# RoboEden/flatland-marl

Measured on AMD Instinct MI355X. Metric: agent-steps/sec (batched envs) + tree-obs build ms/step, higher is better.
Workload: dtype int32; 1 GPU; cfg2: 256 envs x 30x30 / 20 agents / 3 cities (Round-2 Test_2); envs_per_gpu=256, agents=20, obs=cutils(31 nodes, pred 500) + upstream tree depth 2 (pred 30), actions=counter-hash uniform 0..4 generated on device, auto-reset at episode end, distinct_maps=8, dm_rebuild=at commit only, parallelism=envs sharded over 1 GPU(s), metrics all-reduce only, launch=one host call per kernel launch

## Files before the change

flatland_marl_amd/csrc/fl_obs_body.h:

```cpp
#pragma once
#include "fl_obs_trees.h"

__device__ __forceinline__ int obs_env_of_workgroup(const FlObsScratch &S) { return __builtin_amdgcn_readfirstlane(S.order ? S.order[blockIdx.x] : (int)blockIdx.x); }

template <bool CUTILS, int VAR, int STAGE, int MERGED = 0, int FIX = 0, bool UP = true>
__device__ __forceinline__ void obs_body(const FlDev &d, const FlObsScratch &S, const ObsArgs &P_launch) {
    using FixT = ObsFixed<FIX != 0 ? FIX : 1>;
    ObsArgs P_local = P_launch;
    if (FIX != 0) {
        P_local.max_nodes = FixT::max_nodes; P_local.pred_depth = FixT::pred_depth; P_local.tree_pred = FixT::shape.tree_pred;
        P_local.tshift = obs_fixed_tshift<FIX != 0 ? FIX : 1>(d.A);
        if (FixT::max_depth != 0) {
            P_local.max_depth = FixT::max_depth;
            P_local.n_tree_nodes = FixT::max_depth == 2 ? 21 : 85;
        }
    }
    const ObsArgs &P = P_local;
    constexpr bool TAB_LDS = (VAR & 1) != 0, WL_HBM = (VAR & 2) != 0;
    const int b = MERGED == 1 ? (int)blockIdx.x : obs_env_of_workgroup(S), tid = threadIdx.x,
              nt = MERGED == 3 ? 512 : (FIX != 0 || MERGED == 1 || MERGED == 2) ? OBS_NT : (int)blockDim.x;
    const int A = (FIX != 0 && FixT::agents != 0) ? FixT::agents : d.A, R = d.R[b], NS = R * 4, K = d.K[b], U = d.U[b];
    const int Rcap = d.Rcap, Scap = Rcap * 4;
    const int lane = tid & 63, wave = tid >> 6;

// ... 352 lines not shown
            } else va |= 1u << ACT_NOTHING;
        } else if (state == ST_READY) va = (1u << ACT_FORWARD) | (1u << ACT_STOP);
        else va = 1u << ACT_NOTHING;
        if (gl < 5) out_store(&P.valid[(size_t)g * 5 + gl], (uint8_t)((va >> gl) & 1));
        if (P.props && gl == 5) {
            out_store(&P.props[(size_t)g * 3 + 0], (double)dist_target);
            out_store(&P.props[(size_t)g * 3 + 2], (double)(state == ST_READY));
        }
        const int road_type = raw.road_type;
        const uint32_t malfw = raw.malfw;
        const uint32_t malf01 = (malfw & 0xFFFFu) != 0, nmalf01 = (malfw >> 16) != 0;
        const uint32_t rev = __brev(cell) >> 16;
        unsigned long long m_lo = (state < 7u ? 1ull << state : 0ull) | (road_type < 11 ? 1ull << (7 + road_type) : 0ull) | (1ull << (18 + nmalf01)) |
                                  (1ull << (28 + init_dir)) | (1ull << (32 + dir)) | (1ull << (36 + old_dir)) |
                                  ((unsigned long long)(state == ST_MOVING) << 40) | ((unsigned long long)PK_SIGMALF(pk) << 42) |
                                  ((unsigned long long)(!malf01) << 43) | ((unsigned long long)(scount == 0) << 44) |
                                  ((unsigned long long)(scount == max_count) << 45) | ((unsigned long long)(state == ST_MALF || state == ST_MALF_OFF) << 46) |
                                  ((unsigned long long)is_off_map(state) << 47) | ((unsigned long long)is_on_map(state) << 48) |
                                  ((unsigned long long)(rev & 0x7FFFu) << 49);
        const uint32_t m_hi = (rev >> 15) | (va << 1);
        const float max_t = (float)T, max_dist_target = (float)((d.H + d.W) * 8);
        const float f_step = (float)tnow / max_t;
        const float f_latest = (float)raw.latest / max_t;
        const float f_before = f_latest - f_step;
        const float f_dist = isinf(dist_target) ? 8.0f : dist_target / max_dist_target;
        const float fv[13] = {(float)i / (float)A, f_step, (float)raw.earliest / max_t, f_latest, (float)raw.arrival / max_t, f_before, f_dist,
                              f_before < f_dist ? f_before : f_dist, (float)max_count / 10, (float)a_speed[i] / 1.0f, (float)scount / 10,
                              (float)malf01 / 10, isinf(init_dist) ? 8.0f : init_dist / max_dist_target};
        float *o = P.attr + (size_t)g * FL_CUTILS_ATTR;
        out_store(&o[gl], (float)((m_lo >> gl) & 1ull));
        if (gl + 32 != 41) out_store(&o[gl + 32], (float)((m_lo >> (gl + 32)) & 1ull));
        if (gl + 64 < FL_CUTILS_ATTR) {
            float v = (float)((m_hi >> gl) & 1u);
#pragma unroll
            for (int k = 0; k < 13; k++) v = gl == 6 + k ? fv[k] : v;
            out_store(&o[gl + 64], v);
        }
    };
    auto phase1b_all = [&]() __attribute__((always_inline)) {
        for (int i = wave * 2 + (lane >> 5); i < A; i += 2 * (nt >> 6)) phase1b(i, lane & 31, phase1b_load(i));
    };

    const bool do_p1 = CUTILS && STAGE != 2;
    const int nw_walk = (X.Tn > 0 && STAGE != 2) ? min((nt >> 6) - ((do_p1 && (nt >> 6) > 4) ? 1 : 0), max(2, (A + 7) / 8)) : 0;
    const bool p1_beside_walk = nw_walk < (nt >> 6);
    const int n_p1_all = (do_p1 && p1_beside_walk && X.Tn > 0) ? (A + 1) / 2 : 0;
    const bool late_p1 = merged && n_p1_all > 0;
    const int n_up_jobs = (merged && UP) ? (min(A, ROUND) + 3) / 4 : 0, n_p1_jobs = late_p1 ? 0 : n_p1_all;
    constexpr int PF_CHUNK = 64 * 16;
    const int pf_n2 = bg_prefill ? A * P.n_tree_nodes * 6 : 0, n_pf_jobs = (pf_n2 + PF_CHUNK - 1) / PF_CHUNK;
    auto drain_jobs = [&]() __attribute__((always_inline)) {
        bool stored = false;
        while (n_up_jobs + n_p1_jobs + n_pf_jobs > 0) {
            int j = 0;
            if (lane == 0) j = atomicAdd(&misc[6], 1);
            j = __builtin_amdgcn_readfirstlane(j);
            if (j >= n_up_jobs + n_p1_jobs + n_pf_jobs) break;
            if (j < n_up_jobs) {
                const int u = 4 * j + (lane >> 4);
                upstream_pass_a<16, OBS_CAP_T_COMPACT, true, 32>(X, P, b, u, u < A, lane & 15, merged_table_t<ROUND>(wave_scr, min(u, ROUND - 1)), &d.err[b]);
            } else if (j < n_up_jobs + n_p1_jobs) {
                const int i = 2 * (j - n_up_jobs) + (lane >> 5);
                if (i < A) phase1b(i, lane & 31, phase1b_load(i));
            } else {
                double2 *o2 = reinterpret_cast<double2 *>(P.tree_out + (size_t)b * A * P.n_tree_nodes * 12);
                const double2 ninf = make_double2(-INFINITY, -INFINITY);
                const int k0 = (j - n_up_jobs - n_p1_jobs) * PF_CHUNK + lane;
#pragma unroll
                for (int q = 0; q < 16; q++)
                    if (k0 + q * 64 < pf_n2) fill_store_d2(reinterpret_cast<double *>(o2 + k0 + q * 64), -INFINITY, -INFINITY);
                stored = true;
            }
        }
        if (stored) asm volatile("s_waitcnt vmcnt(0)" ::: "memory");
    };
    constexpr bool TOPO_JOBS = MERGED == 1 && OBS_TOPO_JOBS;
    auto late_jobs = [&](bool after_barrier = false) __attribute__((always_inline)) {
        while (late_p1 && !(TOPO_JOBS && after_barrier)) {
            int j = 0;
            if (lane == 0) j = atomicAdd(&misc[7], 1);
            j = __builtin_amdgcn_readfirstlane(j);
            if (j >= n_p1_all) break;
            const int i = 2 * j + (lane >> 5);
            if (i < A) phase1b(i, lane & 31, phase1b_load(i));
        }
        while (TOPO_JOBS && (after_barrier || P.no_early_topo == 0)) {
            int j = 0;
            if (lane == 0) j = atomicAdd(&misc[5], 1);
            j = __builtin_amdgcn_readfirstlane(j);
            if (2 * j >= min(A, 32)) break;
            const int t = 2 * j + (lane >> 5);
            const bool have_t = t < A;
            cutils_rows_orders<OBS_CAP_C, !UP, 1>(X, d, P, b, t, have_t, lane & 31, merged_table_c(wave_scr, min(t, 31)),
                                                  have_t ? team_meta[64 + t] : 1, have_t ? team_meta[192 + t] : 0, (float)T);
        }
    };
    if (do_p1 && (!p1_beside_walk || X.Tn == 0)) {
        if (wave == 0) phase1a();
        phase1b_all();
        __syncthreads();
    }
    OBS_STAMP(2);
    if (X.Tn > 0) {
        const bool dual = UP && CUTILS && STAGE == 1 && p_dual_index && P.tree_pred >= 0;
        const bool reuse = STAGE == 2 && p_dual_index && misc[4] != 0;
        const int Tn2 = P.tree_pred + 1, tshift2 = Tn2 <= 64 ? 0 : P.tshift;
        const bool bk = CUTILS && STAGE != 2 && p_bk != 0 && X.Tn > 64 && X.tmask != nullptr;
        const bool bk_lds = bk && p_bk == 2;
        const int bk_nb = p_bk_nb, bk_shift = p_bk_shift;
        const int bk_w = bk_lds ? bk_nb + 2 : bk_nb;
        uint32_t *bkc = bk_lds ? LDS_AT(uint32_t, L_BKREL) : reinterpret_cast<uint32_t *>(wave_scr);
        if (!reuse) {
            for (int k = tid; k <= K; k += nt) csr[k] = 0;
            if (tid == 0) misc[11] = 0;
            if (X.tmask) for (int k = tid; k <= K; k += nt) { tmask[k] = 0ull; if (X.tmask_m2) tmask_m2[k] = 0ull; }
            if (cmask) for (int k = tid; k < NS; k += nt) cmask[k] = 0ull;
            if (bk) for (int k = tid; k < (bk_lds ? K * bk_w / 2 : ((K + 1) * bk_nb + 1) / 2); k += nt) bkc[k] = 0u;
        }
        if (dual) for (int k = tid; k <= K; k += nt) { csr2[k] = 0; if (p_use_tmask) tmaskb[k] = 0ull; if (X.tmask_m2) tmaskb_m2[k] = 0ull; }
        if (dual && cmaskb) for (int k = tid; k < NS; k += nt) cmaskb[k] = 0u;
        if (STAGE != 2 && tid < 64) { team_meta[64 + tid] = 1; team_meta[192 + tid] = 1; }
        __syncthreads();
        const int pred_depth = my_pred_depth;
        if (STAGE != 2) {
        const int w_first = (nt >> 6) - nw_walk, wsel = wave - w_first;
        if (do_p1 && p1_beside_walk && wave == w_first - 1) {
            phase1a();
#ifdef FL_OBS_TIMING
            if (lane == 0) atomicMax((unsigned long long *)&X.dbg[20], (unsigned long long)wall_clock64());
#endif
        }
        if (wsel >= 0) __builtin_amdgcn_s_setprio(3);
        const int n_max = CUTILS ? pred_depth + 1 : max(pred_depth, 1);
        for (int base = 0; wsel >= 0 && base < A; base += 8 * nw_walk) {
            const int slot = lane >> 3, j = lane & 7;
            const int i = base + wsel * 8 + slot;
            const bool have = i < A;
            const int ia = have ? i : 0;
            uint16_t *path = S.path + ((size_t)b * A + ia) * OBS_PRED_CAP;
            const int u = a_tslot[ia];
            uint32_t st = ((uint32_t)a_vpos[ia] << 2) | a_dir[ia];
            bool alive = have && j < n_max;
            auto lead_in = [&](const uint16_t *nh_u) __attribute__((always_inline)) {
                for (int h = 0; h < 7; h++) {
                    if (alive && h < j) {
                        const uint32_t hop = ((uint32_t)nh_u[st >> 2] >> (3u * (st & 3u))) & 7u;
                        const uint32_t nr = hop == 4u ? (uint32_t)FL_R_NONE : (uint32_t)nbr[(st & ~3u) | hop];
                        if (nr == FL_R_NONE) alive = false;
                        else st = (nr << 2) | hop;
                    }
                }
            };
            const bool listed = !lab || lab[ia] >= 0;
            const int hz1 = ((bk && !bk_lds) || !listed) ? -1 : max(0, CUTILS ? (X.Tn - 2) / (int)a_tpc[ia] + 1 : (X.Tn - 1) / (int)a_tpc[ia]);
            const int tpc_w = a_tpc[ia], tlast_w = X.Tn - 1;
            uint32_t st_hz = 0;
            const int hz2 = dual ? max(0, min(P.tree_pred - 1, (Tn2 - 1) / (int)a_tpc2[ia])) : -1;
            auto walk8 = [&](const uint16_t *h8) __attribute__((always_inline)) {
                int idx = j, last = -1;
                while (__any(alive)) {
                    if (alive) {
                        path[idx] = (uint16_t)st;
                        last = idx;
                        if (idx <= hz1 || idx <= hz2) {
                            const int key = key_of(X, (int)(st >> 2));
                            if (idx <= hz1) {
                                if (bk_lds) {
                                    const int tlo = idx == 0 ? 0 : (idx - 1) * tpc_w + 1, thi = min(idx * tpc_w, tlast_w);
                                    const int b1 = min(tlo >> bk_shift, bk_nb - 1), b2 = min(thi >> bk_shift, bk_nb - 1);
                                    for (int bb = b1; bb <= b2; bb++) {
                                        const int kb = key * bk_w + bb;
                                        atomicAdd(&bkc[kb >> 1], (kb & 1) ? 0x10000u : 1u);
                                    }
                                    atomicAdd(&csr[key], b2 - b1 + 1);
                                    if (idx == hz1) st_hz = st;
                                } else {
                                    atomicAdd(&csr[key], 1);
                                }
                            }
                            if (idx <= hz2) atomicAdd(&csr2[key], 1);
                        }
                        const uint32_t s8 = idx + 8 < n_max ? (uint32_t)h8[st] : (uint32_t)FL_R_NONE;
                        if (s8 == FL_R_NONE) alive = false;
                        else { st = s8; idx += 8; }
                    }
                }
                return last;
            };
            if (nh_in_lds) lead_in(nh_lds + u * Rcap);
            else lead_in(gnh + (size_t)u * Rcap);
            const int my_last = TAB_LDS ? walk8(hop8_lds + u * Scap) : walk8(ghop8 + (size_t)u * Scap);
            int m = my_last;
            m = max(m, __shfl_xor(m, 1)); m = max(m, __shfl_xor(m, 2)); m = max(m, __shfl_xor(m, 4));
            if (bk_lds && have && listed) {
                const int lp = max(0, min(m, hz1));
                if (lp == m ? my_last == lp : j == (lp & 7)) {
                    const uint32_t s_lp = lp == m ? st : st_hz;
                    const int key = key_of(X, (int)(s_lp >> 2));
                    const int tlo = lp == 0 ? 0 : (lp - 1) * tpc_w + 1, thi = min(lp * tpc_w, tlast_w);
                    const int b1 = min(tlo >> bk_shift, bk_nb - 1), b2 = min(thi >> bk_shift, bk_nb - 1);
                    for (int bb = b1; bb <= b2; bb++) {
                        const int kb = key * bk_w + bb;
                        atomicSub(&bkc[kb >> 1], (kb & 1) ? 0x10000u : 1u);
                    }
                    atomicAdd(&bkc[(key * bk_w + bk_nb) >> 1], 1u);
                    atomicOr(&bkc[(key * bk_w + bk_nb) >> 1], 0x10000u << (b1 >> OBS_FB_MSHIFT));
                    if (b2 > b1) atomicSub(&csr[key], b2 - b1);
                }
            }
            if (have && j == 0) {
                const int n = m + 1;
                const int tpc = a_tpc[i];
                const int horizon = CUTILS ? (X.Tn - 2) / tpc + 1 : (X.Tn - 1) / tpc;
                a_lp[i] = (uint16_t)max(0, min(n - 1, horizon));
                a_n[i] = (uint16_t)n;
                if (dual) {
                    const int tpc2 = a_tpc2[i];
                    const int n_py = (n - 1 < P.tree_pred) ? n : P.tree_pred;
                    a_lp2[i] = (uint16_t)max(0, min(n_py - 1, (Tn2 - 1) / tpc2));
                }
            }
        }
        if (wsel >= 0) __builtin_amdgcn_s_setprio(0);
#ifdef FL_OBS_TIMING
        if (wsel >= 0 && lane == 0) atomicMax((unsigned long long *)&X.dbg[21], (unsigned long long)wall_clock64());
#endif
        {
#ifdef FL_OBS_TIMING
            const long long t_pa0 = (long long)wall_clock64();
#endif
            if (CUTILS && (!bk || bk_lds) && P.max_nodes <= OBS_CAP_C) {
                const int n_first = min(A, merged ? ROUND : (nt >> 6) * 2);
                auto hoisted = [&](auto team_tag) __attribute__((always_inline)) {
                    constexpr int TEAM = decltype(team_tag)::value;
                    const int grp = lane / TEAM, gl = lane % TEAM, team_id = wave * (64 / TEAM) + grp;
                    if (__builtin_amdgcn_readfirstlane(wave * (64 / TEAM)) >= n_first) return;
                    int node_base, levels;
                    const bool have = team_id < n_first;
                    cutils_pass_a<OBS_CAP_C, TEAM>(X, d, P, b, team_id, have, grp, gl,
                                  merged ? merged_table_c(wave_scr, min(team_id, ROUND - 1)) : wave_scr + min(team_id, min((nt >> 6) * 2, A)) * (N_WORDS_C * OBS_CAP_C),
                                  a_vpos, a_pos, a_dir, a_state, a_speed, a_tslot, (float)T,
                                  a_raw ? a_raw[(have ? team_id : 0) * 8 + 1] : d.spk[b * A + (have ? team_id : 0)],
                                  a_raw ? a_raw[(have ? team_id : 0) * 8 + 2] : d.malf[b * A + (have ? team_id : 0)], node_base, levels);
                    if (gl == 0 && have) { team_meta[64 + team_id] = node_base; team_meta[192 + team_id] = levels; }
                };
                if (p_compact_t) hoisted(std::integral_constant<int, 16>());
                else hoisted(std::integral_constant<int, 32>());
            }
#ifdef FL_OBS_TIMING
            if (lane == 0) {
                atomicMax((unsigned long long *)&X.dbg[19], (unsigned long long)wall_clock64());
                atomicMax((unsigned long long *)&X.dbg[23], (unsigned long long)((long long)wall_clock64() - t_pa0));
            }
#endif
            drain_jobs();
        }
#ifdef FL_OBS_TIMING
        if (lane == 0) atomicMax((unsigned long long *)&X.dbg[22], (unsigned long long)wall_clock64());
#endif
        if (bk && !bk_lds) {
            __syncthreads();
            for (int i = wave; i < A; i += (nt >> 6)) {
                if (lab && lab[i] < 0) continue;
                const uint16_t *path = S.path + ((size_t)b * A + i) * OBS_PRED_CAP;
                const int lp = a_lp[i];
                const int tpc = a_tpc[i], tlast = X.Tn - 1;
                for (int k0 = lane; k0 <= lp; k0 += 256) {
                    uint32_t wv[4];
#pragma unroll
                    for (int q = 0; q < 4; q++) wv[q] = path[min(k0 + 64 * q, lp)];
#pragma unroll
                    for (int q = 0; q < 4; q++) {
                        const int k = k0 + 64 * q;
                        if (k > lp) break;
                        const int key = key_of(X, (int)(wv[q] >> 2));
                        const int tlo = k == 0 ? 0 : (k - 1) * tpc + 1, span = k == 0 ? 1 : tpc;
                        const int thi = (k == lp || tlo + span - 1 >= tlast) ? tlast : tlo + span - 1;
                        const int b1 = min(tlo >> bk_shift, bk_nb - 1), b2 = min(thi >> bk_shift, bk_nb - 1);
                        for (int bb = b1; bb <= b2; bb++) {
                            const int kb = bb * (K + 1) + key + 1;
                            atomicAdd(&bkc[kb >> 1], (kb & 1) ? 0x10000u : 1u);
                        }
                    }
                }
            }
        }
        } else if (!reuse) {
            for (int i = tid; i < A; i += nt) {
                const int n_c = a_n[i];
                const int n_py = (n_c - 1 < pred_depth) ? n_c : pred_depth;
                const int horizon = (X.Tn - 1) / a_tpc[i];
                a_lp[i] = (uint16_t)max(0, min(n_py - 1, horizon));
            }
            __syncthreads();
            for (int i = wave; i < A; i += (nt >> 6)) {
                const uint16_t *path = S.path + ((size_t)b * A + i) * OBS_PRED_CAP;
                const int lp = a_lp[i];
                for (int k = lane; k <= lp; k += 64) atomicAdd(&csr[key_of(X, (int)(path[k] >> 2))], 1);
            }
        }
        __syncthreads();
        OBS_STAMP(3);
        const bool bk_major = bk && !bk_lds;
        if (!reuse && !bk_major) {
            const int chunk = (K + 1 + nt - 1) / nt;
            const int lo = min(tid * chunk, K + 1), hi = min(lo + chunk, K + 1);
            int sum = 0;
            int longest = 0;
            for (int k = lo; k < hi; k++) {
                sum += dual ? (csr[k] | (csr2[k] << 16)) : csr[k];
                longest = max(longest, dual ? max(csr[k], csr2[k]) : csr[k]);
            }
            if (longest > CF_DIRECT && !bk) misc[11] = 1;
            partial[tid] = sum;
            __syncthreads();
            if (wave == 0) {
                constexpr int PER = OBS_NT / 64;
                const int per = nt >> 6;
                int loc[PER], tot = 0;
#pragma unroll
                for (int q = 0; q < PER; q++) { loc[q] = q < per ? partial[lane * per + q] : 0; tot += loc[q]; }
                const int incl = wave_incl_scan<64>(tot);
                int run = incl - tot;
#pragma unroll
                for (int q = 0; q < PER; q++) { if (q < per) partial[lane * per + q] = run; run += loc[q]; }
            }
            __syncthreads();
            int run = partial[tid];
            if (dual) {
                for (int k = lo; k < hi; k++) {
                    const int v = csr[k] | (csr2[k] << 16);
                    csr[k] = run & 0xFFFF; csr2[k] = (int)((unsigned)run >> 16);
                    run += v;
                }
                if (hi == K + 1 && lo < hi) { misc[2] = run & 0xFFFF; misc[3] = (int)((unsigned)run >> 16); }
            } else {
                for (int k = lo; k < hi; k++) { const int v = csr[k]; csr[k] = run; run += v; }
                if (hi == K + 1 && lo < hi) misc[2] = run;
            }
        }
        if (bk_major) {
            uint16_t *c16 = reinterpret_cast<uint16_t *>(bkc);
            const int K1 = K + 1, n = K1 * bk_nb;
            {
                int most = 0;
                for (int key = tid; key < K; key += nt) {
                    int prev = 0;
                    for (int bb = 0; bb < bk_nb; bb++) { const int c = c16[bb * K1 + key + 1]; most = max(most, prev + c); prev = c; }
                }
                if (most > CF_DIRECT) misc[11] = 1;
            }
            const int chunk = (n + nt - 1) / nt;
            const int lo = min(tid * chunk, n), hi = min(lo + chunk, n);
            int sum = 0;
            for (int k = lo; k < hi; k++) sum += c16[k];
            partial[tid] = sum;
            __syncthreads();
            if (wave == 0) {
                constexpr int PER = OBS_NT / 64;
                const int per = nt >> 6;
                int loc[PER], tot = 0;
#pragma unroll
                for (int q = 0; q < PER; q++) { loc[q] = q < per ? partial[lane * per + q] : 0; tot += loc[q]; }
                const int incl = wave_incl_scan<64>(tot);
                int run = incl - tot;
#pragma unroll
                for (int q = 0; q < PER; q++) { if (q < per) partial[lane * per + q] = run; run += loc[q]; }
            }
            __syncthreads();
            {
                int run = partial[tid];
                for (int k = lo; k < hi; k++) {
                    if (k % K1 == 0) misc[12 + k / K1] = run;
                    run += c16[k];
                }
                if (hi == n && lo < hi) misc[2] = run;
            }
            __syncthreads();
            {
                int run = partial[tid], row = lo / K1, rbase = lo < n ? misc[12 + row] : 0, next = (row + 1) * K1;
                for (int k = lo; k < hi; k++) {
                    if (k == next) { row++; rbase = misc[12 + row]; next += K1; }
                    const int c = c16[k];
                    c16[k] = (uint16_t)(run - rbase);
                    run += c;
                }
            }
        }
        __syncthreads();
        if (reuse) {
            csr = csr2; X.csr_end = csr2; X.items_lds = items2;
            X.tmask = p_use_tmask ? tmaskb : nullptr;
            if (!X.tmask) { X.wl_occ_cap = wl_entries; X.wl_cf = X.wl_occ + X.wl_occ_cap; X.wl_cf_cap = 0; }
        }
        if (bk_lds) {
            for (int key = tid; key < K; key += nt) {
                uint32_t *w4 = bkc + key * (bk_w / 2);
                uint32_t run = 0, prev = 0, most = 0;
                for (int q = 0; q < bk_nb / 2; q++) {
                    const uint32_t v = w4[q], c0 = v & 0xFFFFu, c1 = v >> 16;
                    most = max(most, max(prev + c0 + c1, c0 + c1));
                    prev = c0 + c1;
                    w4[q] = run | ((run + c0) << 16);
                    run += c0 + c1;
                }
                if (bk_lds) {
                    const uint32_t ve = w4[bk_nb / 2];
                    w4[bk_nb / 2] = run | (ve & 0xFFFF0000u);
                    most += ve & 0xFFFFu;
                }
                if (most > CF_DIRECT) misc[11] = 1;
            }
            __syncthreads();
        }
#ifdef FL_OBS_TIMING
        if (STAGE != 2) { __syncthreads(); if (tid == 0) P.dbg[(size_t)b * 64 + 56] = (long long)wall_clock64(); }
#endif
        const bool fit = items_lds != nullptr && misc[2] <= L_FIELD(items_cap);
        const bool dual_fill = dual && misc[3] <= L_FIELD(items2_cap);
        if (dual && tid == 0) misc[4] = dual_fill ? 1 : 0;
        if (merged && UP && !dual_fill) atomicCAS(&d.err[b], 0, FL_ERR_CAPACITY);
        if (fit && !reuse) { csr_items = items_lds; X.items_lds = items_lds; }
        constexpr int FU = 4;
#ifdef OBS_NO_LEAN_FILL
        constexpr bool LEAN_FILL = false;
#else
        constexpr bool LEAN_FILL = MERGED == 1;
#endif
        uint32_t pfv[FU] = {0, 0, 0, 0}, pfn[FU] = {0, 0, 0, 0}, pfp[FU] = {0, 0, 0, 0};
        auto prefetch = [&](int ia) __attribute__((always_inline)) {
            if (reuse || ia >= A) return;
            const uint16_t *pth = S.path + ((size_t)b * A + ia) * OBS_PRED_CAP;
            const int lpn = a_lp[ia];
#pragma unroll
            for (int q = 0; q < FU; q++) {
                const int k = min(lane + 64 * q, lpn);
                pfv[q] = pth[k]; pfn[q] = pth[min(k + 1, lpn)]; pfp[q] = pth[max(k - 1, 0)];
            }
        };
        if (bk_major) {
            const int K1 = K + 1, tlast = X.Tn - 1;
            uint16_t *pre16 = reinterpret_cast<uint16_t *>(partial);
            uint16_t *klo16 = pre16 + ((A + 2) & ~1);
            for (int bb = 0; bb < bk_nb; bb++) {
                const int t0 = bb << bk_shift, t1 = bb == bk_nb - 1 ? tlast : min(t0 + (1 << bk_shift) - 1, tlast);
                if (t0 > tlast) break;
                const int gbase = misc[12 + bb];
                for (int ia = tid; ia < A; ia += nt) {
                    const int lp = a_lp[ia], tpc = a_tpc[ia];
                    const int k_lo = min((t0 + tpc - 1) / tpc, lp);
                    const int k_hi = min(t1 >= 1 ? (t1 - 1) / tpc + 1 : 0, lp);
                    klo16[ia] = (uint16_t)k_lo;
                    pre16[ia + 1] = (lab && lab[ia] < 0) ? (uint16_t)0 : (uint16_t)(k_hi - k_lo + 1);
                }
                if (tid == 0) pre16[0] = 0;
                __syncthreads();
                if (wave == 0) {
                    const int per = (A + 63) >> 6, a_lo = min(lane * per, A), a_hi = min(a_lo + per, A);
                    int sum = 0;
                    for (int ia = a_lo; ia < a_hi; ia++) sum += pre16[ia + 1];
                    int run = wave_incl_scan<64>(sum) - sum;
                    for (int ia = a_lo; ia < a_hi; ia++) { run += pre16[ia + 1]; pre16[ia + 1] = (uint16_t)run; }
                }
                __syncthreads();
                const int total = pre16[A];
                uint32_t nv = 0, nn = 0, np = 0;
                int n_i = 0, n_k = 0;
                auto request = [&](int t) __attribute__((always_inline)) {
                    if (t >= total) return;
                    int lo_a = 0, hi_a = A - 1;
                    while (lo_a < hi_a) {
                        const int mid = (lo_a + hi_a + 1) >> 1;
                        if ((int)pre16[mid] <= t) lo_a = mid; else hi_a = mid - 1;
                    }
                    n_i = lo_a;
                    n_k = (int)klo16[lo_a] + (t - (int)pre16[lo_a]);
                    const uint16_t *pth = S.path + ((size_t)b * A + lo_a) * OBS_PRED_CAP;
                    const int lp = a_lp[lo_a];
                    nv = pth[n_k]; nn = pth[min(n_k + 1, lp)]; np = pth[max(n_k - 1, 0)];
                };
                request(tid);
                for (int t = tid; t < total; t += nt) {
                    const int i = n_i, k = n_k;
                    const uint32_t w = nv, wnx = nn, wpv = np;
                    request(t + nt);
                    const int lp = a_lp[i], tpc = a_tpc[i];
                    const int tlo = k == 0 ? 0 : (k - 1) * tpc + 1, span = k == 0 ? 1 : tpc;
                    const bool to_end = k == lp || tlo + span - 1 >= tlast;
                    const int thi = to_end ? tlast : tlo + span - 1;
                    const int b1 = min(tlo >> bk_shift, bk_nb - 1), b2 = min(thi >> bk_shift, bk_nb - 1);
                    if (bb < b1 || bb > b2) continue;
                    const int key = key_of(X, (int)(w >> 2));
                    if (X.tmask && bb == b1) {
                        const int m1 = tb_of(tlo, X.tshift), m2 = tb_of(thi, X.tshift);
                        atomicOr(&tmask[key], ((2ull << m2) - 1ull) & ~((1ull << m1) - 1ull));
                    }
                    const uint32_t dnext = k < lp ? (wnx & 3u) : (w & 3u), dprev = k > 0 ? (wpv & 3u) : (w & 3u);
                    const uint32_t item = IT_MAKE(lab ? (int)lab[i] : i, tlo, to_end, span, dprev, dnext, w & 3u);
                    const int kb = bb * K1 + key + 1;
                    const uint32_t old = atomicAdd(&bkc[kb >> 1], (kb & 1) ? 0x10000u : 1u);
                    csr_items[gbase + (int)((kb & 1) ? (old >> 16) : (old & 0xFFFFu))] = item;
                }
                __syncthreads();
            }
        }
        prefetch(bk_major ? A : wave);
        for (int i = wave; !reuse && !bk_major && i < A; i += (nt >> 6)) {
            const uint16_t *path = S.path + ((size_t)b * A + i) * OBS_PRED_CAP;
            const int lp = (lab && lab[i] < 0) ? -1 : (int)a_lp[i], tpc = a_tpc[i], tlast = X.Tn - 1;
            const int lp2 = dual_fill ? (int)a_lp2[i] : -1, tpc2 = dual_fill ? (int)a_tpc2[i] : 1;
            uint32_t wv[FU], wnx[FU], wpv[FU];
#pragma unroll
            for (int q = 0; q < FU; q++) { wv[q] = pfv[q]; wnx[q] = pfn[q]; wpv[q] = pfp[q]; }
            prefetch(i + (nt >> 6));
            for (int k0 = lane; k0 <= lp; k0 += 64 * FU) {
            if (k0 != lane) {
#pragma unroll
                for (int q = 0; q < FU; q++) {
                    const int k = min(k0 + 64 * q, lp);
                    wv[q] = path[k]; wnx[q] = path[min(k + 1, lp)]; wpv[q] = path[max(k - 1, 0)];
                }
            }
#pragma unroll
            for (int q = 0; q < FU; q++) {
                const int k = k0 + 64 * q;
                if (k > lp) break;
                const uint32_t w = wv[q];
                const uint32_t dnext = k < lp ? (wnx[q] & 3u) : (w & 3u), dprev = k > 0 ? (wpv[q] & 3u) : (w & 3u);
                int tlo, span;
                if (CUTILS) {
                    tlo = k == 0 ? 0 : (k - 1) * tpc + 1;
                    span = k == 0 ? 1 : tpc;
                } else {
                    tlo = k * tpc;
                    span = tpc;
                }
                const bool to_end = k == lp || tlo + span - 1 >= tlast;
                const int key = key_of(X, (int)(w >> 2));
                if (LEAN_FILL) {
                    const int b1 = tb_of(tlo, X.tshift), b2 = tb_of(to_end ? tlast : tlo + span - 1, X.tshift);
                    const unsigned long long bits = ((2ull << b2) - 1ull) & ~((1ull << b1) - 1ull);
                    const bool second = k <= lp2, done = a_state[i] == ST_DONE;
                    const int tlo2 = k * tpc2, tlast2 = Tn2 - 1;
                    const bool to_end2 = k == lp2 || tlo2 + tpc2 - 1 >= tlast2;
                    unsigned long long bits2 = 0ull, seen = 0ull, seen2 = 0ull;
                    int slot2 = 0;
                    if (X.tmask && X.tmask_m2) seen = atomicOr(&tmask[key], bits);
                    else if (X.tmask) atomicOr(&tmask[key], bits);
                    if (second) {
                        if (p_use_tmask) {
                            const int c1 = tb_of(tlo2, tshift2), c2 = tb_of(to_end2 ? tlast2 : tlo2 + tpc2 - 1, tshift2);
                            bits2 = ((2ull << c2) - 1ull) & ~((1ull << c1) - 1ull);
                            if (X.tmask_m2) seen2 = atomicOr(&tmaskb[key], bits2);
                            else atomicOr(&tmaskb[key], bits2);
                        }
                        slot2 = atomicAdd(&csr2[key], 1);
                    }
                    const uint32_t rail = cw_bits(X, (int)(w >> 2));
                    if (X.tmask && cmask) {
                        const uint32_t dirs = cf_dirs_swar(rail, cf_against(w & 3u) | cf_against(dnext) | cf_against(dprev), done);
#pragma unroll
                        for (uint32_t dw = 0; dw < 4; dw++)
                            if ((dirs >> dw) & 1u) atomicOr(&cmask[((uint32_t)key << 2) | dw], bits);
                    }
                    if (second && p_use_tmask && cmaskb) {
                        const uint32_t dirs = cf_dirs_swar(rail, cf_against(w & 3u), done);
                        const unsigned long long lo32 = (unsigned long long)(uint32_t)bits2;
                        const unsigned long long v01 = ((dirs & 1u) ? lo32 : 0ull) | ((dirs & 2u) ? lo32 << 32 : 0ull);
                        const unsigned long long v23 = ((dirs & 4u) ? lo32 : 0ull) | ((dirs & 8u) ? lo32 << 32 : 0ull);
                        unsigned long long *cb = reinterpret_cast<unsigned long long *>(cmaskb) + ((uint32_t)key << 1);
                        if (v01) atomicOr(&cb[0], v01);
                        if (v23) atomicOr(&cb[1], v23);
                    }
                    const uint32_t item = IT_MAKE(lab ? (int)lab[i] : i, tlo, to_end, span, dprev, dnext, w & 3u);
                    if (bk) {
                        const int thi = to_end ? tlast : tlo + span - 1;
                        int c1 = min(tlo >> bk_shift, bk_nb - 1), c2 = min(thi >> bk_shift, bk_nb - 1);
                        if (bk_lds && to_end) c1 = c2 = bk_nb;
                        for (int bb = c1; bb <= c2; bb++) {
                            const int kb = key * bk_w + bb;
                            const uint32_t old = atomicAdd(&bkc[kb >> 1], (kb & 1) ? 0x10000u : 1u);
                            csr_items[csr[key] + (int)((kb & 1) ? (old >> 16) : (old & 0xFFFFu))] = item;
                        }
                    } else {
                        const int slot = atomicAdd(&csr[key], 1);
                        csr_items[slot] = item;
                    }
                    if (seen & bits) atomicOr(&tmask_m2[key], seen & bits);
                    if (second) {
                        if (seen2 & bits2) atomicOr(&tmaskb_m2[key], seen2 & bits2);
                        items2[slot2] = IT_MAKE(i, tlo2, to_end2, tpc2, dprev, k < lp2 ? dnext : (w & 3u), w & 3u);
                    }
                    continue;
                }
                if (X.tmask) {
                    const int b1 = tb_of(tlo, X.tshift), b2 = tb_of(to_end ? tlast : tlo + span - 1, X.tshift);
                    const unsigned long long bits = ((2ull << b2) - 1ull) & ~((1ull << b1) - 1ull);
                    if (X.tmask_m2) {
                        const unsigned long long seen = atomicOr(&tmask[key], bits);
                        if (seen & bits) atomicOr(&tmask_m2[key], seen & bits);
                    } else {
                        atomicOr(&tmask[key], bits);
                    }
                    if (cmask) {
                        const uint32_t dirs = cf_dirs_of(cw_bits(X, (int)(w >> 2)), cf_against(w & 3u) | cf_against(dnext) | cf_against(dprev), a_state[i] == ST_DONE);
#pragma unroll
                        for (uint32_t dw = 0; dw < 4; dw++)
                            if ((dirs >> dw) & 1u) atomicOr(&cmask[((uint32_t)key << 2) | dw], bits);
                    }
                }
                const uint32_t item = IT_MAKE(lab ? (int)lab[i] : i, tlo, to_end, span, dprev, dnext, w & 3u);
                if (bk) {
                    const int thi = to_end ? tlast : tlo + span - 1;
                    int b1 = min(tlo >> bk_shift, bk_nb - 1), b2 = min(thi >> bk_shift, bk_nb - 1);
                    if (bk_lds && to_end) b1 = b2 = bk_nb;
                    for (int bb = b1; bb <= b2; bb++) {
                        const int kb = key * bk_w + bb;
                        const uint32_t old = atomicAdd(&bkc[kb >> 1], (kb & 1) ? 0x10000u : 1u);
                        csr_items[csr[key] + (int)((kb & 1) ? (old >> 16) : (old & 0xFFFFu))] = item;
                    }
                } else {
                    const int slot = atomicAdd(&csr[key], 1);
                    csr_items[slot] = item;
                }
                if (k <= lp2) {
                    const int tlo2 = k * tpc2, tlast2 = Tn2 - 1;
                    const bool to_end2 = k == lp2 || tlo2 + tpc2 - 1 >= tlast2;
                    const uint32_t dnext2 = k < lp2 ? dnext : (w & 3u);
                    if (p_use_tmask) {
                        const int b1 = tb_of(tlo2, tshift2), b2 = tb_of(to_end2 ? tlast2 : tlo2 + tpc2 - 1, tshift2);
                        const unsigned long long bits = ((2ull << b2) - 1ull) & ~((1ull << b1) - 1ull);
                        if (X.tmask_m2) {
                            const unsigned long long seen = atomicOr(&tmaskb[key], bits);
                            if (seen & bits) atomicOr(&tmaskb_m2[key], seen & bits);
                        } else {
                            atomicOr(&tmaskb[key], bits);
                        }
                        if (cmaskb) {
                            const uint32_t dirs = cf_dirs_of(cw_bits(X, (int)(w >> 2)), cf_against(w & 3u), a_state[i] == ST_DONE);
#pragma unroll
                            for (uint32_t dw = 0; dw < 4; dw++)
                                if ((dirs >> dw) & 1u) atomicOr(&cmaskb[((uint32_t)key << 2) | dw], (uint32_t)bits);
                        }
                    }
                    const int slot2 = atomicAdd(&csr2[key], 1);
                    items2[slot2] = IT_MAKE(i, tlo2, to_end2, tpc2, dprev, dnext2, w & 3u);
                }
            }
            }
        }
        __syncthreads();
#ifdef FL_OBS_TIMING
        if (STAGE != 2 && tid == 0) {
            P.dbg[(size_t)b * 64 + 57] = (long long)wall_clock64();
            int wp = 0;
            for (int i = 0; i < A; i++) wp += a_n[i];
            P.dbg[(size_t)b * 64 + 58] = misc[2];
            P.dbg[(size_t)b * 64 + 59] = wp;
        }
#endif
        if (bk) {
            if (bk_lds) {
                X.csr_end = csr + 1;
                X.bk_rel_lds = reinterpret_cast<const uint16_t *>(bkc);
            } else {
                uint32_t *g = reinterpret_cast<uint32_t *>(S.bk_rel + (size_t)b * (d.Rcap + 1) * OBS_BK_NB);
                for (int k = tid; k < ((K + 1) * bk_nb + 1) / 2; k += nt) g[k] = bkc[k];
                X.bk_rel = S.bk_rel + (size_t)b * (d.Rcap + 1) * OBS_BK_NB;
                X.bk_base = misc + 12;
                X.bk_k1 = K + 1;
                __syncthreads();
            }
        }
    }

    OBS_STAMP(4);
    const float max_dist = (float)T;
    const int nwaves = nt >> 6;
    const bool items_in_lds = X.items_lds != nullptr;
    if (merged) {
        if (items_in_lds) trees_merged<true, MERGED >= 2, ROUND, UP>(X, d, P, b, wave, lane, nwaves, wave_scr, team_meta, a_vpos, a_pos, a_dir, a_state, a_speed, a_tslot, max_dist, late_jobs, (FIX == 1 || FIX == 5 || !UP) ? nullptr : S.rowmask);
        else trees_merged<false, MERGED >= 2, ROUND, UP>(X, d, P, b, wave, lane, nwaves, wave_scr, team_meta, a_vpos, a_pos, a_dir, a_state, a_speed, a_tslot, max_dist, late_jobs, (FIX == 1 || FIX == 5 || !UP) ? nullptr : S.rowmask);
    } else if (CUTILS && STAGE == 0 && FIX == 0 && P.max_nodes > OBS_CAP_C) {
        if (items_in_lds) trees_cutils<true, 64, true>(X, d, P, b, wave, lane, nwaves, wave_scr, team_meta, a_vpos, a_pos, a_dir, a_state, a_speed, a_tslot, max_dist, false);
        else trees_cutils<false, 64, true>(X, d, P, b, wave, lane, nwaves, wave_scr, team_meta, a_vpos, a_pos, a_dir, a_state, a_speed, a_tslot, max_dist, false);
    } else if (CUTILS) {
        if (items_in_lds) trees_cutils<true, OBS_CAP_C, STAGE == 0>(X, d, P, b, wave, lane, nwaves, wave_scr, team_meta, a_vpos, a_pos, a_dir, a_state, a_speed, a_tslot, max_dist, STAGE != 2 && X.Tn > 0 && X.bk_rel == nullptr);
        else trees_cutils<false, OBS_CAP_C, STAGE == 0>(X, d, P, b, wave, lane, nwaves, wave_scr, team_meta, a_vpos, a_pos, a_dir, a_state, a_speed, a_tslot, max_dist, STAGE != 2 && X.Tn > 0 && X.bk_rel == nullptr);
    } else if (p_compact_t && STAGE == 0 && FIX == 0 && P.max_depth >= 4) {
        if (items_in_lds) tree_upstream<32, 32, true, true>(X, d, P, b, wave, lane, nwaves, wave_scr, team_meta, nullptr);
        else tree_upstream<32, 32, true, false>(X, d, P, b, wave, lane, nwaves, wave_scr, team_meta, nullptr);
    } else if (p_compact_t) {
        if (items_in_lds) tree_upstream<16, OBS_CAP_T_COMPACT, true, true>(X, d, P, b, wave, lane, nwaves, wave_scr, team_meta, S.rowmask);
        else tree_upstream<16, OBS_CAP_T_COMPACT, true, false>(X, d, P, b, wave, lane, nwaves, wave_scr, team_meta, S.rowmask);
    } else if (P.max_depth <= 2) {
        if (items_in_lds) tree_upstream<32, 32, false, true>(X, d, P, b, wave, lane, nwaves, wave_scr, team_meta, S.rowmask);
        else tree_upstream<32, 32, false, false>(X, d, P, b, wave, lane, nwaves, wave_scr, team_meta, S.rowmask);
    } else {
        if (items_in_lds) tree_upstream<64, 88, false, true>(X, d, P, b, wave, lane, nwaves, wave_scr, team_meta, S.rowmask);
        else tree_upstream<64, 88, false, false>(X, d, P, b, wave, lane, nwaves, wave_scr, team_meta, S.rowmask);
    }
    OBS_STAMP(5);
#undef LDS_AT
#undef LDS_OPT
}

template <int MODE, int VAR, int FIX>
__device__ __forceinline__ void obs_kernel_body(const FlDev &d, const FlObsScratch &S, const ObsArgs &P) {
    if (MODE != 3 && MODE != 6 && S.order && threadIdx.x == 0) {
        extern __shared__ __align__(16) unsigned char lds[];
        int *misc = reinterpret_cast<int *>(lds + (FIX != 0 ? ObsFixed<FIX != 0 ? FIX : 1>::L.off[L_MISC] : P.L.off[L_MISC]));
        misc[62] = obs_env_of_workgroup(S);
        misc[63] = (int)(uint32_t)wall_clock64();
    }
    if (MODE == 0) obs_body<true, VAR, 0, 0, FIX>(d, S, P);
    else if (MODE == 1) obs_body<false, VAR, 0>(d, S, P);
    else if (MODE == 3) obs_body<true, VAR, 1, 1, FIX>(d, S, P);
    else if (MODE == 4) obs_body<true, VAR, 1, 2, FIX>(d, S, P);
    else if (MODE == 5) obs_body<true, VAR, 1, 3, FIX>(d, S, P);
    else if (MODE == 6) obs_body<true, VAR, 1, 1, FIX, false>(d, S, P);
    else if (MODE == 7) obs_body<true, VAR, 1, 2, FIX, false>(d, S, P);
    else if (MODE == 8) obs_body<true, VAR, 1, 3, FIX, false>(d, S, P);
    else {
        obs_body<true, VAR, 1, 0, FIX>(d, S, P);
        __syncthreads();
        obs_body<false, VAR, 2, 0, FIX>(d, S, P);
    }
    if (MODE != 3 && MODE != 6 && S.order && threadIdx.x == 0) {
        extern __shared__ __align__(16) unsigned char lds[];
        const int *misc = reinterpret_cast<const int *>(lds + (FIX != 0 ? ObsFixed<FIX != 0 ? FIX : 1>::L.off[L_MISC] : P.L.off[L_MISC]));
        S.cost[misc[62]] = (uint32_t)wall_clock64() - (uint32_t)misc[63];
    }
}
template <int MODE, int VAR, int FIX = 0>
__global__ __launch_bounds__(OBS_NT) void k_obs(FlDev d, FlObsScratch S, ObsArgs P) { obs_kernel_body<MODE, VAR, FIX>(d, S, P); }

template <int MODE, int VAR, int FIX, int FIX2 = 0>
__global__ __launch_bounds__(OBS_NT) void k_obs_split(FlDev d, FlObsScratch S, ObsArgs P) {
    const int b = (MODE == 3 || MODE == 6) ? (int)blockIdx.x : obs_env_of_workgroup(S);
    if (d.R[b] <= ObsFixed<FIX>::dims.Rcap) obs_kernel_body<MODE, VAR, FIX>(d, S, P);
    else obs_kernel_body<MODE, VAR, FIX2>(d, S, P);
}
```

Measured before the change: 131.1 million agent-steps/s.

## Flatten lean CSR fill over (agent, path-step) items with early path prefetch

In the merged (MERGED==1) lean-fill path, the per-agent wave loop is replaced by a flat loop over all (agent, step) pairs. The pairs are indexed through a wave-wide inclusive scan of path lengths, so each lane handles one item and short paths no longer leave lanes idle. The first batch of path words is requested before the CSR prefix-sum phase to hide global load latency, and each iteration prefetches the next batch. The scan assumes A ≤ 64 agents and adds per-item scalar readlane search work.

```diff
diff --git a/flatland_marl_amd/csrc/fl_obs_body.h b/flatland_marl_amd/csrc/fl_obs_body.h
--- a/flatland_marl_amd/csrc/fl_obs_body.h
+++ b/flatland_marl_amd/csrc/fl_obs_body.h
@@ -678,6 +678,54 @@
         __syncthreads();
         OBS_STAMP(3);
         const bool bk_major = bk && !bk_lds;
+#ifdef OBS_NO_LEAN_FILL
+        constexpr bool LEAN_FILL = false;
+#else
+        constexpr bool LEAN_FILL = MERGED == 1;
+#endif
+#ifdef OBS_NO_FLAT_FILL
+        constexpr bool FLAT_FILL = false;
+#else
+        constexpr bool FLAT_FILL = LEAN_FILL;
+#endif
+#ifdef FL_OBS_TIMING
+        long long fill_t0_ = 0;
+#define FILL_MARK_T0() do { fill_t0_ = (long long)wall_clock64(); } while (0)
+#define FILL_MARK_WAIT(first) do { if (LEAN_FILL && (first)) { asm volatile("s_waitcnt vmcnt(0)" ::: "memory"); \
+            if (lane == 0) atomicMax((unsigned long long *)&X.dbg[35], (unsigned long long)((long long)wall_clock64() - fill_t0_)); } } while (0)
+#define FILL_MARK_BODY(first) do { if (LEAN_FILL && (first) && lane == 0) atomicMax((unsigned long long *)&X.dbg[33], (unsigned long long)wall_clock64()); } while (0)
+#define FILL_MARK_END() do { if (LEAN_FILL && lane == 0) atomicMax((unsigned long long *)&X.dbg[34], (unsigned long long)wall_clock64()); } while (0)
+#else
+#define FILL_MARK_T0() do {} while (0)
+#define FILL_MARK_WAIT(first) do {} while (0)
+#define FILL_MARK_BODY(first) do {} while (0)
+#define FILL_MARK_END() do {} while (0)
+#endif
+        int ff_incl = 0, ff_total = 0, ff_i = 0, ff_k = 0, ff_lp = 0;
+        uint32_t ff_w = 0, ff_wn = 0, ff_wp = 0;
+        auto ff_request = [&](int t) __attribute__((always_inline)) {
+            const int t_first = __builtin_amdgcn_readfirstlane(t);
+            const int a_lo = __popcll(__ballot(ff_incl <= t_first)), a_hi = min(__popcll(__ballot(ff_incl <= t_first + 63)), A - 1);
+            int i = a_lo, start = a_lo > 0 ? __builtin_amdgcn_readlane(ff_incl, max(a_lo - 1, 0)) : 0;
+            for (int a = a_lo; a < a_hi; a++) {
+                const int e = __builtin_amdgcn_readlane(ff_incl, a);
+                const bool c = e <= t;
+                i += c ? 1 : 0;
+                start = c ? e : start;
+            }
+            ff_i = i; ff_k = t - start;
+            if (t < ff_total) {
+                const uint16_t *pth = S.path + ((size_t)b * A + i) * OBS_PRED_CAP;
+                const int lpn = a_lp[i], k = t - start;
+                ff_lp = lpn;
+                ff_w = pth[k]; ff_wn = pth[min(k + 1, lpn)]; ff_wp = pth[max(k - 1, 0)];
+            }
+        };
+        if (FLAT_FILL && !bk_major) {
+            ff_incl = wave_incl_scan<64>(lane < A ? (int)a_lp[lane] + 1 : 0);
+            ff_total = __builtin_amdgcn_readlane(ff_incl, 63);
+            if ((wave << 6) < ff_total) ff_request(tid);
+        }
         if (!reuse && !bk_major) {
             const int chunk = (K + 1 + nt - 1) / nt;
             const int lo = min(tid * chunk, K + 1), hi = min(lo + chunk, K + 1);
@@ -798,11 +846,6 @@
         if (merged && UP && !dual_fill) atomicCAS(&d.err[b], 0, FL_ERR_CAPACITY);
         if (fit && !reuse) { csr_items = items_lds; X.items_lds = items_lds; }
         constexpr int FU = 4;
-#ifdef OBS_NO_LEAN_FILL
-        constexpr bool LEAN_FILL = false;
-#else
-        constexpr bool LEAN_FILL = MERGED == 1;
-#endif
         uint32_t pfv[FU] = {0, 0, 0, 0}, pfn[FU] = {0, 0, 0, 0}, pfp[FU] = {0, 0, 0, 0};
         auto prefetch = [&](int ia) __attribute__((always_inline)) {
             if (reuse || ia >= A) return;
@@ -814,6 +857,86 @@
                 pfv[q] = pth[k]; pfn[q] = pth[min(k + 1, lpn)]; pfp[q] = pth[max(k - 1, 0)];
             }
         };
+        auto lean_item = [&](int i, int k, int lp, int tpc, int lp2, int tpc2, uint32_t w, uint32_t wn, uint32_t wp) __attribute__((always_inline)) {
+            const int tlast = X.Tn - 1;
+            const uint32_t dnext = k < lp ? (wn & 3u) : (w & 3u), dprev = k > 0 ? (wp & 3u) : (w & 3u);
+            int tlo, span;
+            if (CUTILS) {
+                tlo = k == 0 ? 0 : (k - 1) * tpc + 1;
+                span = k == 0 ? 1 : tpc;
+            } else {
+                tlo = k * tpc;
+                span = tpc;
+            }
+            const bool to_end = k == lp || tlo + span - 1 >= tlast;
+            const int key = key_of(X, (int)(w >> 2));
+            const int b1 = tb_of(tlo, X.tshift), b2 = tb_of(to_end ? tlast : tlo + span - 1, X.tshift);
+            const unsigned long long bits = ((2ull << b2) - 1ull) & ~((1ull << b1) - 1ull);
+            const bool second = k <= lp2, done = a_state[i] == ST_DONE;
+            const int tlo2 = k * tpc2, tlast2 = Tn2 - 1;
+            const bool to_end2 = k == lp2 || tlo2 + tpc2 - 1 >= tlast2;
+            unsigned long long bits2 = 0ull, seen = 0ull, seen2 = 0ull;
+            int slot2 = 0;
+            if (X.tmask && X.tmask_m2) seen = atomicOr(&tmask[key], bits);
+            else if (X.tmask) atomicOr(&tmask[key], bits);
+            if (second) {
+                if (p_use_tmask) {
+                    const int c1 = tb_of(tlo2, tshift2), c2 = tb_of(to_end2 ? tlast2 : tlo2 + tpc2 - 1, tshift2);
+                    bits2 = ((2ull << c2) - 1ull) & ~((1ull << c1) - 1ull);
+                    if (X.tmask_m2) seen2 = atomicOr(&tmaskb[key], bits2);
+                    else atomicOr(&tmaskb[key], bits2);
+                }
+                slot2 = atomicAdd(&csr2[key], 1);
+            }
+            const uint32_t rail = cw_bits(X, (int)(w >> 2));
+            if (X.tmask && cmask) {
+                const uint32_t dirs = cf_dirs_swar(rail, cf_against(w & 3u) | cf_against(dnext) | cf_against(dprev), done);
+#pragma unroll
+                for (uint32_t dw = 0; dw < 4; dw++)
+                    if ((dirs >> dw) & 1u) atomicOr(&cmask[((uint32_t)key << 2) | dw], bits);
+            }
+            if (second && p_use_tmask && cmaskb) {
+                const uint32_t dirs = cf_dirs_swar(rail, cf_against(w & 3u), done);
+                const unsigned long long lo32 = (unsigned long long)(uint32_t)bits2;
+                const unsigned long long v01 = ((dirs & 1u) ? lo32 : 0ull) | ((dirs & 2u) ? lo32 << 32 : 0ull);
+                const unsigned long long v23 = ((dirs & 4u) ? lo32 : 0ull) | ((dirs & 8u) ? lo32 << 32 : 0ull);
+                unsigned long long *cb = reinterpret_cast<unsigned long long *>(cmaskb) + ((uint32_t)key << 1);
+                if (v01) atomicOr(&cb[0], v01);
+                if (v23) atomicOr(&cb[1], v23);
+            }
+            const uint32_t item = IT_MAKE(lab ? (int)lab[i] : i, tlo, to_end, span, dprev, dnext, w & 3u);
+            if (bk) {
+                const int thi = to_end ? tlast : tlo + span - 1;
+                int c1 = min(tlo >> bk_shift, bk_nb - 1), c2 = min(thi >> bk_shift, bk_nb - 1);
+                if (bk_lds && to_end) c1 = c2 = bk_nb;
+                for (int bb = c1; bb <= c2; bb++) {
+                    const int kb = key * bk_w + bb;
+                    const uint32_t old = atomicAdd(&bkc[kb >> 1], (kb & 1) ? 0x10000u : 1u);
+                    csr_items[csr[key] + (int)((kb & 1) ? (old >> 16) : (old & 0xFFFFu))] = item;
+                }
+            } else {
+                const int slot = atomicAdd(&csr[key], 1);
+                csr_items[slot] = item;
+            }
+            if (seen & bits) atomicOr(&tmask_m2[key], seen & bits);
+            if (second) {
+                if (seen2 & bits2) atomicOr(&tmaskb_m2[key], seen2 & bits2);
+                items2[slot2] = IT_MAKE(i, tlo2, to_end2, tpc2, dprev, k < lp2 ? dnext : (w & 3u), w & 3u);
+            }
+        };
+        if (FLAT_FILL && !bk_major) {
+            FILL_MARK_T0();
+            for (int t0 = wave << 6; t0 < ff_total; t0 += nt) {
+                const int i = ff_i, k = ff_k, lp = ff_lp;
+                const uint32_t w = ff_w, wn = ff_wn, wp = ff_wp;
+                FILL_MARK_WAIT(t0 == wave << 6);
+                if (t0 + nt < ff_total) ff_request(t0 + nt + lane);
+                if (t0 + lane < ff_total)
+                    lean_item(i, k, lp, a_tpc[i], dual_fill ? (int)a_lp2[i] : -1, dual_fill ? (int)a_tpc2[i] : 1, w, wn, wp);
+                FILL_MARK_BODY(t0 == wave << 6);
+            }
+            FILL_MARK_END();
+        }
         if (bk_major) {
             const int K1 = K + 1, tlast = X.Tn - 1;
             uint16_t *pre16 = reinterpret_cast<uint16_t *>(partial);
@@ -880,14 +1003,15 @@
                 __syncthreads();
             }
         }
-        prefetch(bk_major ? A : wave);
-        for (int i = wave; !reuse && !bk_major && i < A; i += (nt >> 6)) {
+        if (!FLAT_FILL) { FILL_MARK_T0(); prefetch(bk_major ? A : wave); }
+        for (int i = wave; !FLAT_FILL && !reuse && !bk_major && i < A; i += (nt >> 6)) {
             const uint16_t *path = S.path + ((size_t)b * A + i) * OBS_PRED_CAP;
             const int lp = (lab && lab[i] < 0) ? -1 : (int)a_lp[i], tpc = a_tpc[i], tlast = X.Tn - 1;
             const int lp2 = dual_fill ? (int)a_lp2[i] : -1, tpc2 = dual_fill ? (int)a_tpc2[i] : 1;
             uint32_t wv[FU], wnx[FU], wpv[FU];
 #pragma unroll
             for (int q = 0; q < FU; q++) { wv[q] = pfv[q]; wnx[q] = pfn[q]; wpv[q] = pfp[q]; }
+            FILL_MARK_WAIT(i == wave);
             prefetch(i + (nt >> 6));
             for (int k0 = lane; k0 <= lp; k0 += 64 * FU) {
             if (k0 != lane) {
@@ -914,59 +1038,7 @@
                 const bool to_end = k == lp || tlo + span - 1 >= tlast;
                 const int key = key_of(X, (int)(w >> 2));
                 if (LEAN_FILL) {
-                    const int b1 = tb_of(tlo, X.tshift), b2 = tb_of(to_end ? tlast : tlo + span - 1, X.tshift);
-                    const unsigned long long bits = ((2ull << b2) - 1ull) & ~((1ull << b1) - 1ull);
-                    const bool second = k <= lp2, done = a_state[i] == ST_DONE;
-                    const int tlo2 = k * tpc2, tlast2 = Tn2 - 1;
-                    const bool to_end2 = k == lp2 || tlo2 + tpc2 - 1 >= tlast2;
-                    unsigned long long bits2 = 0ull, seen = 0ull, seen2 = 0ull;
-                    int slot2 = 0;
-                    if (X.tmask && X.tmask_m2) seen = atomicOr(&tmask[key], bits);
-                    else if (X.tmask) atomicOr(&tmask[key], bits);
-                    if (second) {
-                        if (p_use_tmask) {
-                            const int c1 = tb_of(tlo2, tshift2), c2 = tb_of(to_end2 ? tlast2 : tlo2 + tpc2 - 1, tshift2);
-                            bits2 = ((2ull << c2) - 1ull) & ~((1ull << c1) - 1ull);
-                            if (X.tmask_m2) seen2 = atomicOr(&tmaskb[key], bits2);
-                            else atomicOr(&tmaskb[key], bits2);
-                        }
-                        slot2 = atomicAdd(&csr2[key], 1);
-                    }
-                    const uint32_t rail = cw_bits(X, (int)(w >> 2));
-                    if (X.tmask && cmask) {
-                        const uint32_t dirs = cf_dirs_swar(rail, cf_against(w & 3u) | cf_against(dnext) | cf_against(dprev), done);
-#pragma unroll
-                        for (uint32_t dw = 0; dw < 4; dw++)
-                            if ((dirs >> dw) & 1u) atomicOr(&cmask[((uint32_t)key << 2) | dw], bits);
-                    }
-                    if (second && p_use_tmask && cmaskb) {
-                        const uint32_t dirs = cf_dirs_swar(rail, cf_against(w & 3u), done);
-                        const unsigned long long lo32 = (unsigned long long)(uint32_t)bits2;
-                        const unsigned long long v01 = ((dirs & 1u) ? lo32 : 0ull) | ((dirs & 2u) ? lo32 << 32 : 0ull);
-                        const unsigned long long v23 = ((dirs & 4u) ? lo32 : 0ull) | ((dirs & 8u) ? lo32 << 32 : 0ull);
-                        unsigned long long *cb = reinterpret_cast<unsigned long long *>(cmaskb) + ((uint32_t)key << 1);
-                        if (v01) atomicOr(&cb[0], v01);
-                        if (v23) atomicOr(&cb[1], v23);
-                    }
-                    const uint32_t item = IT_MAKE(lab ? (int)lab[i] : i, tlo, to_end, span, dprev, dnext, w & 3u);
-                    if (bk) {
-                        const int thi = to_end ? tlast : tlo + span - 1;
-                        int c1 = min(tlo >> bk_shift, bk_nb - 1), c2 = min(thi >> bk_shift, bk_nb - 1);
-                        if (bk_lds && to_end) c1 = c2 = bk_nb;
-                        for (int bb = c1; bb <= c2; bb++) {
-                            const int kb = key * bk_w + bb;
-                            const uint32_t old = atomicAdd(&bkc[kb >> 1], (kb & 1) ? 0x10000u : 1u);
-                            csr_items[csr[key] + (int)((kb & 1) ? (old >> 16) : (old & 0xFFFFu))] = item;
-                        }
-                    } else {
-                        const int slot = atomicAdd(&csr[key], 1);
-                        csr_items[slot] = item;
-                    }
-                    if (seen & bits) atomicOr(&tmask_m2[key], seen & bits);
-                    if (second) {
-                        if (seen2 & bits2) atomicOr(&tmaskb_m2[key], seen2 & bits2);
-                        items2[slot2] = IT_MAKE(i, tlo2, to_end2, tpc2, dprev, k < lp2 ? dnext : (w & 3u), w & 3u);
-                    }
+                    lean_item(i, k, lp, tpc, lp2, tpc2, w, wnx[q], wpv[q]);
                     continue;
                 }
                 if (X.tmask) {
@@ -1024,7 +1096,9 @@
                 }
             }
             }
-        }
+            FILL_MARK_BODY(i == wave);
+        }
+        if (!FLAT_FILL) FILL_MARK_END();
         __syncthreads();
 #ifdef FL_OBS_TIMING
         if (STAGE != 2 && tid == 0) {
```

After: 134.9 million agent-steps/s, median of 6. +2.9%, better.
